# openai/Video-Pre-Training

Measured on NVIDIA H100. Metric: frames/sec MinecraftPolicy fwd, 128x128x3 BxT=128x128, higher is better.
Workload: dtype bf16

## Files before the change

video-pre-training_b200/csrc/common.cuh:

```cuda
#pragma once
#include <cuda.h>
#include <cuda_bf16.h>
#include <cuda_runtime.h>
#include <stdint.h>

#include "../../include/vpt_b200.h"

namespace vpt {

void set_error(const char* fmt, ...);
#define VPT_CHECK(cond, ...)                 \
    do {                                     \
        if (!(cond)) {                       \
            vpt::set_error(__VA_ARGS__);     \
            return VPT_ERR_ARG;              \
        }                                    \
    } while (0)
#define VPT_CUDA(expr)                                                                   \
    do {                                                                                 \
        cudaError_t _e = (expr);                                                         \
        if (_e != cudaSuccess) {                                                         \
            vpt::set_error("%s failed: %s (%s:%d)", #expr, cudaGetErrorString(_e), __FILE__, __LINE__); \
            return VPT_ERR_CUDA;                                                         \
        }                                                                                \
    } while (0)
#define VPT_LAUNCH_CHECK() VPT_CUDA(cudaGetLastError())
static int g_pdl = 0;
template <typename... KArgs, typename... Args>
static inline void launch_k(void (*kernel)(KArgs...), dim3 grid, dim3 block, size_t smem, cudaStream_t stream, Args&&... args) {
    cudaLaunchConfig_t cfg;
    memset(&cfg, 0, sizeof(cfg));
    cfg.gridDim = grid;
    cfg.blockDim = block;
    cfg.dynamicSmemBytes = smem;
    cfg.stream = stream;
    cudaLaunchAttribute attr[1];
    attr[0].id = cudaLaunchAttributeProgrammaticStreamSerialization;
    attr[0].val.programmaticStreamSerializationAllowed = 1;
    cfg.attrs = attr;
    cfg.numAttrs = g_pdl ? 1 : 0;
    (void)cudaLaunchKernelEx(&cfg, kernel, static_cast<KArgs>(args)...);
}


#ifndef VPT_NO_WATCHDOG
__device__ unsigned int g_device_error = 0;
#endif

__device__ __forceinline__ void pdl_sync() {
    asm volatile("griddepcontrol.launch_dependents;" ::: "memory");
    asm volatile("griddepcontrol.wait;" ::: "memory");
}
__device__ __forceinline__ uint32_t smem_u32(const void* p) { return (uint32_t)__cvta_generic_to_shared(p); }
__device__ __forceinline__ int lane_id() { return threadIdx.x & 31; }

__device__ __forceinline__ float warp_sum(float v) {
#pragma unroll
    for (int o = 16; o > 0; o >>= 1) v += __shfl_xor_sync(0xffffffffu, v, o);
    return v;
}
__device__ __forceinline__ float warp_max(float v) {
#pragma unroll
    for (int o = 16; o > 0; o >>= 1) v = fmaxf(v, __shfl_xor_sync(0xffffffffu, v, o));
    return v;
}

__device__ __forceinline__ uint32_t pack_bf16(float lo, float hi) {
    __nv_bfloat162 v = __floats2bfloat162_rn(lo, hi);
    return *reinterpret_cast<uint32_t*>(&v);
}
__device__ __forceinline__ float bf16_lo(uint32_t v) { return __uint_as_float(v << 16); }
__device__ __forceinline__ float bf16_hi(uint32_t v) { return __uint_as_float(v & 0xffff0000u); }
__device__ __forceinline__ float round_bf16(float v) { return __bfloat162float(__float2bfloat16_rn(v)); }

__device__ __forceinline__ void mbar_init(uint64_t* bar, uint32_t count) {
    asm volatile("mbarrier.init.shared::cta.b64 [%0], %1;" ::"r"(smem_u32(bar)), "r"(count));
}
__device__ __forceinline__ void fence_barrier_init() { asm volatile("fence.mbarrier_init.release.cluster;" ::: "memory"); }
__device__ __forceinline__ void fence_proxy_async() { asm volatile("fence.proxy.async.shared::cta;" ::: "memory"); }
__device__ __forceinline__ void mbar_expect_tx(uint64_t* bar, uint32_t bytes) {
    asm volatile("mbarrier.arrive.expect_tx.shared::cta.b64 _, [%0], %1;" ::"r"(smem_u32(bar)), "r"(bytes) : "memory");
}
__device__ __forceinline__ void mbar_arrive(uint64_t* bar) {
    asm volatile("mbarrier.arrive.shared::cta.b64 _, [%0];" ::"r"(smem_u32(bar)) : "memory");
}
__device__ __forceinline__ bool mbar_try_wait(uint64_t* bar, uint32_t parity) {
    uint32_t ok;
    asm volatile(
        "{\n\t.reg .pred p;\n\t"
        "mbarrier.try_wait.parity.shared::cta.b64 p, [%1], %2;\n\t"
        "selp.b32 %0, 1, 0, p;\n\t}"
        : "=r"(ok)
        : "r"(smem_u32(bar)), "r"(parity)
        : "memory");
    return ok != 0;
}
__device__ __forceinline__ bool mbar_try_wait_sleep(uint64_t* bar, uint32_t parity, uint32_t ns) {
    uint32_t ok;
    asm volatile(
        "{\n\t.reg .pred p;\n\t"
        "mbarrier.try_wait.parity.shared::cta.b64 p, [%1], %2, %3;\n\t"
        "selp.b32 %0, 1, 0, p;\n\t}"
        : "=r"(ok)
        : "r"(smem_u32(bar)), "r"(parity), "r"(ns)
        : "memory");
    return ok != 0;
}
__device__ __forceinline__ bool mbar_wait(uint64_t* bar, uint32_t parity, unsigned int code) {
    if (mbar_try_wait(bar, parity)) return true;
    const long long t0 = clock64();
    for (unsigned int it = 1;; ++it) {
        if (mbar_try_wait_sleep(bar, parity, 20000u)) return true;
        if ((it & 63u) == 0u) {
            if (*(volatile unsigned int*)&g_device_error != 0u) return false;
            if (clock64() - t0 > 3000000000LL) {
                atomicCAS(&g_device_error, 0u, code);
                return false;
            }
        }
    }
}

__device__ __forceinline__ void tma_prefetch_desc(const CUtensorMap* m) {
    asm volatile("prefetch.tensormap [%0];" ::"l"((uint64_t)m) : "memory");
}
__device__ __forceinline__ void tma_load_2d(void* dst, const CUtensorMap* m, uint64_t* bar, int c0, int c1) {
    asm volatile(
        "cp.async.bulk.tensor.2d.shared::cluster.global.tile.mbarrier::complete_tx::bytes [%0], [%1, {%3, %4}], [%2];" ::"r"(
            smem_u32(dst)),
        "l"((uint64_t)m), "r"(smem_u32(bar)), "r"(c0), "r"(c1)
        : "memory");
}
__device__ __forceinline__ void tma_load_4d(void* dst, const CUtensorMap* m, uint64_t* bar, int c0, int c1, int c2, int c3) {
    asm volatile(
        "cp.async.bulk.tensor.4d.shared::cluster.global.tile.mbarrier::complete_tx::bytes [%0], [%1, {%3, %4, %5, %6}], [%2];" ::"r"(
            smem_u32(dst)),
        "l"((uint64_t)m), "r"(smem_u32(bar)), "r"(c0), "r"(c1), "r"(c2), "r"(c3)
        : "memory");
}

__device__ __forceinline__ void tma_store_2d(const CUtensorMap* m, const void* src, int c0, int c1) {
    asm volatile("cp.async.bulk.tensor.2d.global.shared::cta.bulk_group [%0, {%2, %3}], [%1];" ::"l"((uint64_t)m), "r"(smem_u32(src)), "r"(c0),
                 "r"(c1)
                 : "memory");
}
__device__ __forceinline__ void bulk_commit() { asm volatile("cp.async.bulk.commit_group;" ::: "memory"); }
template <int N>
__device__ __forceinline__ void bulk_wait_read() {
    asm volatile("cp.async.bulk.wait_group.read %0;" ::"n"(N) : "memory");
}
template <int N>
__device__ __forceinline__ void bulk_wait_all() {
    asm volatile("cp.async.bulk.wait_group %0;" ::"n"(N) : "memory");
}
__device__ __forceinline__ void named_bar_sync(int id, int nthreads) { asm volatile("bar.sync %0, %1;" ::"r"(id), "r"(nthreads) : "memory"); }
__device__ __forceinline__ void named_bar_arrive(int id, int nthreads) { asm volatile("bar.arrive %0, %1;" ::"r"(id), "r"(nthreads) : "memory"); }

__device__ __forceinline__ void tma_load_2d_mc(void* dst, const CUtensorMap* m, uint64_t* bar, int c0, int c1, uint16_t cta_mask) {
    asm volatile(
        "cp.async.bulk.tensor.2d.shared::cluster.global.tile.mbarrier::complete_tx::bytes.multicast::cluster [%0], [%1, {%3, %4}], [%2], %5;" ::"r"(
            smem_u32(dst)),
        "l"((uint64_t)m), "r"(smem_u32(bar)), "r"(c0), "r"(c1), "h"(cta_mask)
        : "memory");
}

__device__ __forceinline__ void mbar_arrive_cluster(uint64_t* bar, uint32_t rank) {
    asm volatile(
        "{\n\t.reg .b32 ra;\n\t"
        "mapa.shared::cluster.u32 ra, %0, %1;\n\t"
        "mbarrier.arrive.release.cluster.shared::cluster.b64 _, [ra];\n\t}" ::"r"(smem_u32(bar)),
        "r"(rank)
        : "memory");
}
__device__ __forceinline__ uint32_t cluster_ctarank() {
    uint32_t r;
    asm volatile("mov.u32 %0, %%cluster_ctarank;" : "=r"(r));
    return r;
}
__device__ __forceinline__ void cluster_sync_all() {
    asm volatile("barrier.cluster.arrive.release.aligned;\n\tbarrier.cluster.wait.acquire.aligned;" ::: "memory");
}

__device__ __forceinline__ void wgmma_fence() { asm volatile("wgmma.fence.sync.aligned;" ::: "memory"); }
__device__ __forceinline__ void wgmma_commit() { asm volatile("wgmma.commit_group.sync.aligned;" ::: "memory"); }
template <int N>
__device__ __forceinline__ void wgmma_wait() { asm volatile("wgmma.wait_group.sync.aligned %0;" ::"n"(N) : "memory"); }
template <int N>
__device__ __forceinline__ void wgmma_reg_fence(float (&d)[N]) {
#pragma unroll
    for (int i = 0; i < N; ++i) asm volatile("" : "+f"(d[i])::"memory");
}

template <int TA, int TB>
__device__ __forceinline__ void wgmma_n64(float (&d)[32], uint64_t a_desc, uint64_t b_desc, uint32_t accumulate) {
    asm volatile(
        "{\n\t.reg .pred p;\n\t"
        "setp.ne.b32 p, %34, 0;\n\t"
        "wgmma.mma_async.sync.aligned.m64n64k16.f32.bf16.bf16 "
        "{%0, %1, %2, %3, %4, %5, %6, %7, %8, %9, %10, %11, %12, %13, %14, %15, %16, %17, %18, %19, %20, %21, %22, %23, %24, %25, %26, %27, %28, %29, %30, %31}, %32, %33, p, 1, 1, %35, %36;\n\t}"
        : "+f"(d[0]), "+f"(d[1]), "+f"(d[2]), "+f"(d[3]), "+f"(d[4]), "+f"(d[5]), "+f"(d[6]), "+f"(d[7]), "+f"(d[8]), "+f"(d[9]), "+f"(d[10]), "+f"(d[11]), "+f"(d[12]), "+f"(d[13]), "+f"(d[14]), "+f"(d[15]), "+f"(d[16]), "+f"(d[17]), "+f"(d[18]), "+f"(d[19]), "+f"(d[20]), "+f"(d[21]), "+f"(d[22]), "+f"(d[23]), "+f"(d[24]), "+f"(d[25]), "+f"(d[26]), "+f"(d[27]), "+f"(d[28]), "+f"(d[29]), "+f"(d[30]), "+f"(d[31])
        : "l"(a_desc), "l"(b_desc), "r"(accumulate), "n"(TA), "n"(TB)
        : "memory");
}

template <int TA, int TB>
__device__ __forceinline__ void wgmma_n128(float (&d)[64], uint64_t a_desc, uint64_t b_desc, uint32_t accumulate) {
    asm volatile(
        "{\n\t.reg .pred p;\n\t"
        "setp.ne.b32 p, %66, 0;\n\t"
        "wgmma.mma_async.sync.aligned.m64n128k16.f32.bf16.bf16 "
        "{%0, %1, %2, %3, %4, %5, %6, %7, %8, %9, %10, %11, %12, %13, %14, %15, %16, %17, %18, %19, %20, %21, %22, %23, %24, %25, %26, %27, %28, %29, %30, %31, %32, %33, %34, %35, %36, %37, %38, %39, %40, %41, %42, %43, %44, %45, %46, %47, %48, %49, %50, %51, %52, %53, %54, %55, %56, %57, %58, %59, %60, %61, %62, %63}, %64, %65, p, 1, 1, %67, %68;\n\t}"
        : "+f"(d[0]), "+f"(d[1]), "+f"(d[2]), "+f"(d[3]), "+f"(d[4]), "+f"(d[5]), "+f"(d[6]), "+f"(d[7]), "+f"(d[8]), "+f"(d[9]), "+f"(d[10]), "+f"(d[11]), "+f"(d[12]), "+f"(d[13]), "+f"(d[14]), "+f"(d[15]), "+f"(d[16]), "+f"(d[17]), "+f"(d[18]), "+f"(d[19]), "+f"(d[20]), "+f"(d[21]), "+f"(d[22]), "+f"(d[23]), "+f"(d[24]), "+f"(d[25]), "+f"(d[26]), "+f"(d[27]), "+f"(d[28]), "+f"(d[29]), "+f"(d[30]), "+f"(d[31]), "+f"(d[32]), "+f"(d[33]), "+f"(d[34]), "+f"(d[35]), "+f"(d[36]), "+f"(d[37]), "+f"(d[38]), "+f"(d[39]), "+f"(d[40]), "+f"(d[41]), "+f"(d[42]), "+f"(d[43]), "+f"(d[44]), "+f"(d[45]), "+f"(d[46]), "+f"(d[47]), "+f"(d[48]), "+f"(d[49]), "+f"(d[50]), "+f"(d[51]), "+f"(d[52]), "+f"(d[53]), "+f"(d[54]), "+f"(d[55]), "+f"(d[56]), "+f"(d[57]), "+f"(d[58]), "+f"(d[59]), "+f"(d[60]), "+f"(d[61]), "+f"(d[62]), "+f"(d[63])
        : "l"(a_desc), "l"(b_desc), "r"(accumulate), "n"(TA), "n"(TB)
        : "memory");
}

template <int R>
__device__ __forceinline__ void setmaxnreg_dec() { asm volatile("setmaxnreg.dec.sync.aligned.u32 %0;" ::"n"(R)); }
template <int R>
__device__ __forceinline__ void setmaxnreg_inc() { asm volatile("setmaxnreg.inc.sync.aligned.u32 %0;" ::"n"(R)); }

__device__ __forceinline__ uint64_t gmma_desc_sw128(uint32_t smem_addr, uint32_t lbo_bytes = 16u, uint32_t sbo_bytes = 1024u) {
    uint64_t d = 0;
    d |= (uint64_t)((smem_addr & 0x3FFFFu) >> 4);
    d |= (uint64_t)(lbo_bytes >> 4) << 16;
    d |= (uint64_t)(sbo_bytes >> 4) << 32;
    d |= (uint64_t)1 << 62;
    return d;
}

template <int NR>
__device__ __forceinline__ void wgmma_frag_store(const float (&d)[NR], float* stg, int pitch, int col0) {
    const int w = (threadIdx.x >> 5) & 3, l = threadIdx.x & 31;
    const int r0 = 16 * w + (l >> 2), c0 = col0 + 2 * (l & 3);
#pragma unroll
    for (int i = 0; i < NR / 4; ++i) {
        *reinterpret_cast<float2*>(stg + (size_t)r0 * pitch + c0 + 8 * i) = make_float2(d[4 * i], d[4 * i + 1]);
        *reinterpret_cast<float2*>(stg + (size_t)(r0 + 8) * pitch + c0 + 8 * i) = make_float2(d[4 * i + 2], d[4 * i + 3]);
    }
}
__device__ __forceinline__ void stg_ld_32(const float* src, uint32_t (&v)[32]) {
#pragma unroll
    for (int q = 0; q < 8; ++q) {
        const float4 x = reinterpret_cast<const float4*>(src)[q];
        v[4 * q] = __float_as_uint(x.x); v[4 * q + 1] = __float_as_uint(x.y); v[4 * q + 2] = __float_as_uint(x.z); v[4 * q + 3] = __float_as_uint(x.w);
    }
}

}
```

video-pre-training_b200/csrc/conv_zp.cuh:

```cuda
#pragma once
#include "common.cuh"
#include "gemm_tc.cuh"

namespace vpt {

static int g_cz_dbg = 0;

constexpr int kCzThreads = 384;
constexpr int kCzMaxBStages = 8;
constexpr int kCzProducerRegs = 24, kCzMmaRegs = 240;

constexpr int kCzBarOrder = 1, kCzBarStg = 3, kCzBarWg = 5;

struct ConvZpParams {
    long long Q;
    int H, W, Wp, FS;
    int N, block_n, num_n_tiles, cin, cin_blocks;
    int a_box_rows, a_boxes, a_stage_bytes, b_stages;
    int dbg;
    int bo;
    long long num_m_tiles;
    const float* mr;
    const float* S1;
    const float* S2;
    int relu;
    const __nv_bfloat16* residual;
    __nv_bfloat16* out;
    float* stat_part;
    const float* Ef;
    const float* res_scale;
    const float* res_shift;
};

template <int BN>
__device__ __forceinline__ void cz_mma_k16(float (&acc)[BN / 2], uint64_t a_desc, uint64_t b_desc, uint32_t accumulate) {
    if constexpr (BN == 128)
        wgmma_n128<0, 0>(acc, a_desc, b_desc, accumulate);
    else
        wgmma_n64<0, 0>(acc, a_desc, b_desc, accumulate);
}

template <int BN>
__global__ void __launch_bounds__(kCzThreads, 1)
conv3x3_zp_kernel(const __grid_constant__ CUtensorMap tmA, const __grid_constant__ CUtensorMap tmB, const ConvZpParams p) {
    static_assert(BN == 64 || BN == 128, "BN is 64 or 128");
    pdl_sync();
    extern __shared__ uint8_t smem_raw[];
    const uint32_t raw = smem_u32(smem_raw);
    uint8_t* smem = smem_raw + (((raw + 1023u) & ~1023u) - raw);
    constexpr uint32_t b_stage_bytes = (uint32_t)BN * kBlockK * 2;
    uint8_t* smem_a = smem;
    uint8_t* smem_b = smem + 2 * (size_t)p.a_stage_bytes;
    float* stg = reinterpret_cast<float*>(smem_b + (size_t)p.b_stages * b_stage_bytes);
    uint64_t* bars = reinterpret_cast<uint64_t*>(reinterpret_cast<uint8_t*>(stg) + kStgBytes);
    uint64_t* a_full = bars;
    uint64_t* a_empty = bars + 2;
    uint64_t* b_full = bars + 4;
    uint64_t* b_empty = bars + 4 + kCzMaxBStages;

    const int warp = threadIdx.x >> 5;
    const int lane = threadIdx.x & 31;

    if (warp == 8 && lane == 0) {
        tma_prefetch_desc(&tmA);
        tma_prefetch_desc(&tmB);
        for (int i = 0; i < 2; ++i) {
            mbar_init(&a_full[i], 1);
            mbar_init(&a_empty[i], 1);
        }
        for (int i = 0; i < p.b_stages; ++i) {
            mbar_init(&b_full[i], 1);
            mbar_init(&b_empty[i], 1);
        }
        fence_barrier_init();
    }
    __syncthreads();

    const int num_tiles = (int)(p.num_m_tiles * p.num_n_tiles);
    const int tile_begin = (int)blockIdx.x;
    const int tile_step = (int)gridDim.x;
    const int halo = p.Wp + 1;

    if (warp >= 8) {
        setmaxnreg_dec<kCzProducerRegs>();
        if (warp == 8 && lane == 0) {
            int stage = 0;
            uint32_t phase = 0;
            bool ok = true;
            for (int tile = tile_begin; tile < num_tiles && ok; tile += tile_step) {
                const int m_tile = tile / p.num_n_tiles;
                const int span0 = m_tile * kBlockM - halo;
                for (int cb = 0; cb < p.cin_blocks; ++cb) {
                    if (!(ok = mbar_wait(&a_empty[stage], phase ^ 1u, 0x110u))) break;
                    mbar_expect_tx(&a_full[stage], (uint32_t)p.a_stage_bytes);
                    uint8_t* sa = smem_a + (size_t)stage * p.a_stage_bytes;
                    for (int b = 0; b < p.a_boxes; ++b)
                        tma_load_2d(sa + (size_t)b * p.a_box_rows * 128, &tmA, &a_full[stage], cb * kBlockK, span0 + b * p.a_box_rows);
                    advance(stage, phase, 2);
                }
            }
        } else if (warp == 9 && lane == 0) {
            int stage = 0;
            uint32_t phase = 0;
            bool ok = true;
            for (int tile = tile_begin; tile < num_tiles && ok; tile += tile_step) {
                const int n0 = (tile % p.num_n_tiles) * BN;
                for (int cb = 0; cb < p.cin_blocks && ok; ++cb) {
                    for (int tap = 0; tap < 9; ++tap) {
                        if (!(ok = mbar_wait(&b_empty[stage], phase ^ 1u, 0x120u))) break;
                        mbar_expect_tx(&b_full[stage], b_stage_bytes);
                        tma_load_2d(smem_b + (size_t)stage * b_stage_bytes, &tmB, &b_full[stage], tap * p.cin + cb * kBlockK, n0);
                        advance(stage, phase, p.b_stages);
                    }
                }
            }
        }
        return;
    }

    setmaxnreg_inc<kCzMmaRegs>();
    const int wg = warp >> 2;
    const int wwarp = warp & 3;
    float* my_row = stg + (size_t)(wwarp * 32 + lane) * kStgPitch;
    const int nchunks = BN >> 5;
    const int c_half = (nchunks + 1) >> 1;
    const int P = p.num_n_tiles * 2;
    const bool res_vec = (((uintptr_t)p.residual | (uintptr_t)p.res_scale | (uintptr_t)p.res_shift) & 15) == 0;
    const int b_per_tile = 9 * p.cin_blocks;
    for (int s = wg; tile_begin + s * tile_step < num_tiles; s += 2) {
        const int tile = tile_begin + s * tile_step;
        const bool has_next = tile + tile_step < num_tiles;
        const int m_tile = tile / p.num_n_tiles;
        const int n_tile = tile % p.num_n_tiles;
        const int n0 = n_tile * BN;
        const long long a_it = (long long)s * p.cin_blocks, b_it = (long long)s * b_per_tile;
        int astage = (int)(a_it & 1), bstage = (int)(b_it % p.b_stages);
        uint32_t aphase = (uint32_t)((a_it >> 1) & 1), bphase = (uint32_t)((b_it / p.b_stages) & 1);

        if (s > 0) named_bar_sync(kCzBarOrder + wg, 256);
        float frag[2][BN / 2];
        bool ok = true;
        int prev_b = -1, prev_a = -1;
        for (int cb = 0; cb < p.cin_blocks && ok; ++cb) {
            if (!(ok = mbar_wait(&a_full[astage], aphase, 0x310u))) break;
            const uint32_t a_base = smem_u32(smem_a + (size_t)astage * p.a_stage_bytes);
#pragma unroll 1
            for (int tap = 0; tap < 9; ++tap) {
                if (!(ok = mbar_wait(&b_full[bstage], bphase, 0x320u))) break;
                const uint32_t b_addr = smem_u32(smem_b + (size_t)bstage * b_stage_bytes);
                const int row_off = (tap / 3) * p.Wp + (tap % 3);
                const uint32_t a_addr = a_base + (uint32_t)row_off * 128u;
                const uint64_t a_bo = p.bo ? ((uint64_t)((a_addr >> 7) & 7u) << 49) : 0ull;
                wgmma_fence();
#pragma unroll
                for (int k = 0; k < kBlockK / 16; ++k) {
                    const uint32_t acc = (uint32_t)((cb | tap | k) != 0);
                    const uint64_t bd = gmma_desc_sw128(b_addr + k * 32);
                    cz_mma_k16<BN>(frag[0], gmma_desc_sw128(a_addr + k * 32) | a_bo, bd, acc);
                    cz_mma_k16<BN>(frag[1], gmma_desc_sw128(a_addr + 64u * 128u + k * 32) | a_bo, bd, acc);
                }
                wgmma_commit();
                wgmma_wait<1>();
                if ((threadIdx.x & 127) == 0) {
                    if (prev_b >= 0) mbar_arrive(&b_empty[prev_b]);
                    if (prev_a >= 0) mbar_arrive(&a_empty[prev_a]);
                }
                prev_a = -1;
                prev_b = bstage;
                advance(bstage, bphase, p.b_stages);
            }
            prev_a = astage;
            advance(astage, aphase, 2);
        }
        if (has_next) named_bar_arrive(kCzBarOrder + (wg ^ 1), 256);
        wgmma_wait<0>();
#pragma unroll
        for (int h = 0; h < 2; ++h) wgmma_reg_fence(frag[h]);
        if ((threadIdx.x & 127) == 0) {
            if (prev_b >= 0) mbar_arrive(&b_empty[prev_b]);
            if (prev_a >= 0) mbar_arrive(&a_empty[prev_a]);
        }
        if (!ok) {
            if (has_next) named_bar_arrive(kCzBarStg + (wg ^ 1), 256);
            break;
        }

        if (s > 0) named_bar_sync(kCzBarStg + wg, 256);
#pragma unroll
        for (int h = 0; h < 2; ++h) wgmma_frag_store(frag[h], stg + (size_t)h * 64 * kStgPitch, kStgPitch, 0);
        named_bar_sync(kCzBarWg + wg, 128);

        const int q = m_tile * kBlockM + wwarp * 32 + lane;
        const bool row_ok = q < p.Q;
        const int f = q / p.FS;
        const int r = q - f * p.FS;
        const int y = r / p.Wp, x = r - y * p.Wp;
        const bool interior = row_ok && (y < p.H) && (x < p.W);
        float ga = 1.f, gb = 0.f;
        if (p.mr != nullptr && interior) {
            const float mean = __ldg(p.mr + 2 * f), rstd = __ldg(p.mr + 2 * f + 1);
            ga = rstd;
            gb = rstd * mean;
        }
        const int cy = (y == 0) ? 0 : ((y == p.H - 1) ? 2 : 1);
        const int cx = (x == 0) ? 0 : ((x == p.W - 1) ? 2 : 1);
        const int cls = interior ? cy * 3 + cx : 0;
        const float* s1row = p.S1 ? p.S1 + (size_t)cls * p.N : nullptr;
        const float* s2row = p.S2 ? p.S2 + (size_t)cls * p.N : nullptr;
        if (p.Ef) {
            s1row = nullptr;
            s2row = p.Ef + ((size_t)(interior ? f : 0) * 9 + cls) * p.N;
        }
        const float* rarow = (p.res_scale && interior) ? p.res_scale + (size_t)f * p.N : nullptr;
        const float* rbrow = (p.res_scale && interior) ? p.res_shift + (size_t)f * p.N : nullptr;
        float st_s0 = 0.f, st_ss0 = 0.f, st_s1 = 0.f, st_ss1 = 0.f;

        const int qw = m_tile * kBlockM + wwarp * 32;
        float* wrows = stg + (size_t)(wwarp * 32) * kStgPitch;
        const int seg = lane & 3;
#pragma unroll 1
        for (int c = 0; c < (p.dbg == 2 ? 0 : nchunks); ++c) {
            const int g = c < c_half ? 0 : 1;
            const int nb = n0 + c * 32;
            const int lim = min(32, min(BN - c * 32, p.N - nb));
            if (lim <= 0) break;
            const bool full = (lim == 32) && ((p.N & 7) == 0) && res_vec;
            uint32_t acc[32];
            float v[32];
            uint32_t pk[16];
            if (full) {
                stg_ld_32(my_row + c * 32, acc);
                __syncwarp();
                if (p.residual != nullptr) {
#pragma unroll
                    for (int k = 0; k < 4; ++k) {
                        const int rr = 8 * k + (lane >> 2);
                        if (qw + rr < p.Q)
                            reinterpret_cast<uint4*>(wrows + (size_t)rr * kStgPitch + c * 32)[seg] =
                                __ldg(reinterpret_cast<const uint4*>(p.residual + (size_t)(qw + rr) * p.N + nb) + seg);
                    }
                    __syncwarp();
                }
                if (row_ok) {
                    if (!interior) {
#pragma unroll
                        for (int j = 0; j < 16; ++j) pk[j] = 0u;
                    } else {
#pragma unroll
                        for (int qq = 0; qq < 8; ++qq) {
                            float4 a1 = s1row ? __ldg(reinterpret_cast<const float4*>(s1row + nb) + qq) : make_float4(0, 0, 0, 0);
                            float4 a2 = s2row ? __ldg(reinterpret_cast<const float4*>(s2row + nb) + qq) : make_float4(0, 0, 0, 0);
                            v[4 * qq + 0] = fmaf(ga, __uint_as_float(acc[4 * qq + 0]), fmaf(-gb, a1.x, a2.x));
                            v[4 * qq + 1] = fmaf(ga, __uint_as_float(acc[4 * qq + 1]), fmaf(-gb, a1.y, a2.y));
                            v[4 * qq + 2] = fmaf(ga, __uint_as_float(acc[4 * qq + 2]), fmaf(-gb, a1.z, a2.z));
                            v[4 * qq + 3] = fmaf(ga, __uint_as_float(acc[4 * qq + 3]), fmaf(-gb, a1.w, a2.w));
                        }
                        if (p.relu == 1) {
#pragma unroll
                            for (int j = 0; j < 32; ++j) v[j] = fmaxf(v[j], 0.f);
                        }
                        if (p.residual != nullptr) {
                            const uint4* rp = reinterpret_cast<const uint4*>(my_row + c * 32);
#pragma unroll
                            for (int qq = 0; qq < 4; ++qq) {
                                const uint4 rr = rp[qq];
                                const float r8[8] = {bf16_lo(rr.x), bf16_hi(rr.x), bf16_lo(rr.y), bf16_hi(rr.y),
                                                     bf16_lo(rr.z), bf16_hi(rr.z), bf16_lo(rr.w), bf16_hi(rr.w)};
                                if (rarow) {
                                    const float4* ra4 = reinterpret_cast<const float4*>(rarow + nb) + 2 * qq;
                                    const float4* rb4 = reinterpret_cast<const float4*>(rbrow + nb) + 2 * qq;
                                    const float4 a0 = __ldg(ra4), a1 = __ldg(ra4 + 1), b0 = __ldg(rb4), b1 = __ldg(rb4 + 1);
                                    const float ra[8] = {a0.x, a0.y, a0.z, a0.w, a1.x, a1.y, a1.z, a1.w};
                                    const float rb[8] = {b0.x, b0.y, b0.z, b0.w, b1.x, b1.y, b1.z, b1.w};
#pragma unroll
                                    for (int j = 0; j < 8; ++j) v[8 * qq + j] += fmaf(ra[j], r8[j], rb[j]);
                                } else {
#pragma unroll
                                    for (int j = 0; j < 8; ++j) v[8 * qq + j] += r8[j];
                                }
                            }
                        }
                        if (p.relu == 2) {
#pragma unroll
                            for (int j = 0; j < 32; ++j) v[j] = fmaxf(v[j], 0.f);
                        }
#pragma unroll
                        for (int j = 0; j < 16; ++j) pk[j] = pack_bf16(v[2 * j], v[2 * j + 1]);
                        if (p.stat_part) {
                            float s_ = g ? st_s1 : st_s0, ss_ = g ? st_ss1 : st_ss0;
#pragma unroll
                            for (int j = 0; j < 16; ++j) {
                                const float lo = bf16_lo(pk[j]), hi = bf16_hi(pk[j]);
                                s_ += lo; ss_ = fmaf(lo, lo, ss_);
                                s_ += hi; ss_ = fmaf(hi, hi, ss_);
                            }
                            if (g) { st_s1 = s_; st_ss1 = ss_; } else { st_s0 = s_; st_ss0 = ss_; }
                        }
                    }
#pragma unroll
                    for (int qq = 0; qq < 4; ++qq)
                        reinterpret_cast<uint4*>(my_row + c * 32 + 16)[qq] = make_uint4(pk[4 * qq], pk[4 * qq + 1], pk[4 * qq + 2], pk[4 * qq + 3]);
                }
                __syncwarp();
                if (p.dbg != 1) {
#pragma unroll
                    for (int k = 0; k < 4; ++k) {
                        const int rr = 8 * k + (lane >> 2);
                        if (qw + rr < p.Q)
                            reinterpret_cast<uint4*>(p.out + (size_t)(qw + rr) * p.N + nb)[seg] =
                                reinterpret_cast<const uint4*>(wrows + (size_t)rr * kStgPitch + c * 32 + 16)[seg];
                    }
                }
                continue;
            }
            if (!row_ok) continue;
            stg_ld_32(my_row + c * 32, acc);
            __nv_bfloat16* op = p.out + (size_t)q * p.N + nb;
            if (!interior) {
                for (int j = 0; j < lim; ++j) op[j] = __float2bfloat16_rn(0.f);
                continue;
            }
#pragma unroll
            for (int j = 0; j < 32; ++j) {
                float a1 = 0.f, a2 = 0.f;
                if (j < lim) {
                    if (s1row) a1 = __ldg(s1row + nb + j);
                    if (s2row) a2 = __ldg(s2row + nb + j);
                }
                v[j] = fmaf(ga, __uint_as_float(acc[j]), fmaf(-gb, a1, a2));
            }
            if (p.relu == 1) {
#pragma unroll
                for (int j = 0; j < 32; ++j) v[j] = fmaxf(v[j], 0.f);
            }
            if (p.residual != nullptr) {
                const __nv_bfloat16* rp = p.residual + (size_t)q * p.N + nb;
#pragma unroll
                for (int j = 0; j < 32; ++j)
                    if (j < lim) v[j] += rarow ? fmaf(__ldg(rarow + nb + j), __bfloat162float(rp[j]), __ldg(rbrow + nb + j)) : __bfloat162float(rp[j]);
            }
            if (p.relu == 2) {
#pragma unroll
                for (int j = 0; j < 32; ++j) v[j] = fmaxf(v[j], 0.f);
            }
#pragma unroll
            for (int j = 0; j < 16; ++j) pk[j] = pack_bf16(v[2 * j], v[2 * j + 1]);
            if (p.stat_part) {
                float s_ = g ? st_s1 : st_s0, ss_ = g ? st_ss1 : st_ss0;
#pragma unroll
                for (int j = 0; j < 16; ++j) {
                    const float lo = bf16_lo(pk[j]), hi = bf16_hi(pk[j]);
                    if (2 * j < lim) { s_ += lo; ss_ = fmaf(lo, lo, ss_); }
                    if (2 * j + 1 < lim) { s_ += hi; ss_ = fmaf(hi, hi, ss_); }
                }
                if (g) { st_s1 = s_; st_ss1 = ss_; } else { st_s0 = s_; st_ss0 = ss_; }
            }
            if (p.dbg != 1) {
#pragma unroll
                for (int j = 0; j < 32; ++j)
                    if (j < lim) op[j] = __float2bfloat16_rn(v[j]);
            }
        }
        if (has_next) named_bar_arrive(kCzBarStg + (wg ^ 1), 256);
        if (p.stat_part && row_ok)
            reinterpret_cast<float4*>(p.stat_part)[((size_t)q * P + n_tile * 2) >> 1] = make_float4(st_s0, st_ss0, st_s1, st_ss1);
    }
}

}

namespace vpt {
static inline void conv_zp_block_n(long long Q, int N, int* bn, int* nt) {
    choose_block_n(N, bn, nt);
    const long long tiles = (Q + kBlockM - 1) / kBlockM;
    if (tiles * *nt >= 64 || *bn == 64) return;
    *bn = 64;
    *nt = (N + 63) / 64;
}
}

extern "C" int vpt_conv3x3_zp(const vpt_conv_zp_args* a, void* stream) {
    using namespace vpt;
    VPT_CHECK(a && a->x && a->w && a->out, "vpt_conv3x3_zp: null operand");
    const int H = a->H, W = a->W, C = a->Cin, N = a->Cout;
    VPT_CHECK(a->F > 0 && H >= 2 && W >= 2 && C > 0 && C % 64 == 0 && N > 0 && N % 16 == 0,
              "vpt_conv3x3_zp: need F>0, H,W>=2, Cin %% 64 == 0, Cout %% 16 == 0 (F=%d H=%d W=%d Cin=%d Cout=%d)", a->F, H, W, C, N);
    VPT_CHECK(W <= 182, "vpt_conv3x3_zp: W=%d too wide (at most 182: two input spans of 128 + 2*(W+2) rows must fit in shared memory)", W);
    VPT_CHECK(((uintptr_t)a->x & 15) == 0 && ((uintptr_t)a->w & 15) == 0 && ((uintptr_t)a->out & 15) == 0, "vpt_conv3x3_zp: pointers must be 16-byte aligned");
    ConvZpParams p;
    memset(&p, 0, sizeof(p));
    p.H = H; p.W = W; p.Wp = W + 1; p.FS = (H + 1) * (W + 1);
    p.Q = (long long)a->F * p.FS;
    VPT_CHECK(p.Q <= 2147483647LL - kBlockM, "vpt_conv3x3_zp: too many rows for 32-bit row indices and TMA coordinates");
    p.N = N; p.cin = C; p.cin_blocks = C / 64;
    conv_zp_block_n(p.Q, N, &p.block_n, &p.num_n_tiles);
    p.num_m_tiles = (p.Q + kBlockM - 1) / kBlockM;
    const int span = kBlockM + 2 * (p.Wp + 1);
    p.a_boxes = (span + 255) / 256;
    p.a_box_rows = ((span + p.a_boxes - 1) / p.a_boxes + 7) / 8 * 8;
    VPT_CHECK(p.a_box_rows <= 256, "vpt_conv3x3_zp: span does not fit the TMA box limit");
    p.a_stage_bytes = p.a_boxes * p.a_box_rows * 128;
    const uint32_t b_stage_bytes = (uint32_t)p.block_n * kBlockK * 2;
    const size_t fixed_bytes = 1024 + 2 * (size_t)p.a_stage_bytes + kStgBytes + (4 + 2 * kCzMaxBStages) * 8;
    int bst = (int)((227 * 1024 - (long long)fixed_bytes) / b_stage_bytes);
    if (bst > kCzMaxBStages) bst = kCzMaxBStages;
    VPT_CHECK(bst >= 2, "vpt_conv3x3_zp: not enough shared memory for the weight pipeline (W=%d Cout=%d)", W, N);
    p.b_stages = bst;
    const size_t smem_bytes = fixed_bytes + (size_t)bst * b_stage_bytes;

    CUtensorMap tmA, tmB;
    {
        cuuint64_t dims[2] = {(cuuint64_t)C, (cuuint64_t)p.Q};
        cuuint64_t strides[1] = {(cuuint64_t)C * 2};
        cuuint32_t box[2] = {64, (cuuint32_t)p.a_box_rows};
        int r = make_tmap_bf16(&tmA, a->x, 2, dims, strides, box);
        if (r) return r;
    }
    {
        cuuint64_t dims[2] = {(cuuint64_t)9 * C, (cuuint64_t)N};
        cuuint64_t strides[1] = {(cuuint64_t)9 * C * 2};
        cuuint32_t box[2] = {64, (cuuint32_t)p.block_n};
        int r = make_tmap_bf16(&tmB, a->w, 2, dims, strides, box);
        if (r) return r;
    }
    VPT_CHECK(!(a->mr && !a->S1 && !a->Ef), "vpt_conv3x3_zp: mr given without S1 (or Ef)");
    VPT_CHECK(!a->Ef || a->mr, "vpt_conv3x3_zp: Ef needs mr = (0, rstd) per frame");
    VPT_CHECK(!a->res_scale == !a->res_shift && (!a->res_scale || a->residual) && (!a->res_scale || N % 8 == 0),
              "vpt_conv3x3_zp: res_scale / res_shift come as a pair, with a residual, Cout %% 8 == 0");
    p.mr = a->mr; p.S1 = a->mr ? a->S1 : nullptr; p.S2 = a->S2; p.relu = a->relu;
    p.residual = reinterpret_cast<const __nv_bfloat16*>(a->residual);
    p.out = reinterpret_cast<__nv_bfloat16*>(a->out);
    p.stat_part = a->stat_part;
    p.Ef = a->Ef; p.res_scale = a->res_scale; p.res_shift = a->res_shift;
    p.dbg = g_cz_dbg;
    p.bo = g_dbg_bo > 0 ? 1 : 0;

    static bool attr_set = false;
    if (!attr_set) {
        VPT_CUDA(cudaFuncSetAttribute(conv3x3_zp_kernel<64>, cudaFuncAttributeMaxDynamicSharedMemorySize, 227 * 1024));
        VPT_CUDA(cudaFuncSetAttribute(conv3x3_zp_kernel<128>, cudaFuncAttributeMaxDynamicSharedMemorySize, 227 * 1024));
        attr_set = true;
    }
    const long long tiles = p.num_m_tiles * p.num_n_tiles;
    long long grid = num_sms();
    if (grid <= 0) grid = 132;
    if (grid > tiles) grid = tiles;
    if (p.block_n == 64)
        launch_k(conv3x3_zp_kernel<64>, dim3((unsigned)grid), dim3(kCzThreads), smem_bytes, (cudaStream_t)stream, tmA, tmB, p);
    else
        launch_k(conv3x3_zp_kernel<128>, dim3((unsigned)grid), dim3(kCzThreads), smem_bytes, (cudaStream_t)stream, tmA, tmB, p);
    VPT_LAUNCH_CHECK();
    return VPT_OK;
}

extern "C" int vpt_set_conv_pair_mode(int32_t on) {
    vpt::g_cz_dbg = (on & 0xff) >> 4;
    return VPT_OK;
}

extern "C" int vpt_set_conv_swap_mode(int32_t on) {
    (void)on;
    return VPT_OK;
}

extern "C" int64_t vpt_conv_zp_t_stat_floats(int32_t F, int32_t H, int32_t W, int32_t Cout) {
    (void)F; (void)H; (void)W; (void)Cout;
    return 0;
}

extern "C" int vpt_conv_zp_t_stats_finalize(const float* part, float* mr, int32_t F, int32_t H, int32_t W, float eps, void* stream) {
    (void)part; (void)mr; (void)F; (void)H; (void)W; (void)eps; (void)stream;
    vpt::set_error("vpt_conv_zp_t_stats_finalize: no convolution kernel of this build emits per-tile partials (vpt_conv_zp_t_stat_floats is 0)");
    return VPT_ERR_ARG;
}

extern "C" int vpt_conv_zp_stat_parts(int32_t F, int32_t H, int32_t W, int32_t Cout) {
    const long long Q = (long long)F * (H + 1) * (W + 1);
    int bn, nt;
    vpt::conv_zp_block_n(Q, Cout, &bn, &nt);
    return nt * 2;
}
```

Baseline: 26620.

## Stage conv epilogue per warp and chunk instead of whole-tile shared staging

The epilogue of the zero-padded 3x3 conv kernel now gives each warp a private 32-row staging area with a 36-float pitch. Each 32-column chunk of the wgmma fragment is written there on demand, instead of staging the whole tile into a buffer shared by the warpgroup. This removes the inter-warpgroup staging barriers and the warpgroup-wide sync, and shrinks the staging shared memory, which can leave room for more weight pipeline stages. Residual loads for the next chunk are issued early, before the wgmma wait and between chunks, to hide global latency. The cost is more __syncwarp calls, a switch on chunk index, and more live registers for the prefetched residual.

```diff
diff --git a/video-pre-training_b200/csrc/common.cuh b/video-pre-training_b200/csrc/common.cuh
--- a/video-pre-training_b200/csrc/common.cuh
+++ b/video-pre-training_b200/csrc/common.cuh
@@ -239,6 +239,17 @@
         *reinterpret_cast<float2*>(stg + (size_t)(r0 + 8) * pitch + c0 + 8 * i) = make_float2(d[4 * i + 2], d[4 * i + 3]);
     }
 }
+template <int C, int NR>
+__device__ __forceinline__ void wgmma_frag_store_chunk(const float (&d)[NR], float* blk, int pitch) {
+    static_assert(16 * C + 16 <= NR, "chunk outside the fragment");
+    const int l = threadIdx.x & 31;
+    float* dst = blk + (size_t)(l >> 2) * pitch + 2 * (l & 3);
+#pragma unroll
+    for (int i = 0; i < 4; ++i) {
+        *reinterpret_cast<float2*>(dst + 8 * i) = make_float2(d[16 * C + 4 * i], d[16 * C + 4 * i + 1]);
+        *reinterpret_cast<float2*>(dst + (size_t)8 * pitch + 8 * i) = make_float2(d[16 * C + 4 * i + 2], d[16 * C + 4 * i + 3]);
+    }
+}
 __device__ __forceinline__ void stg_ld_32(const float* src, uint32_t (&v)[32]) {
 #pragma unroll
     for (int q = 0; q < 8; ++q) {
diff --git a/video-pre-training_b200/csrc/conv_zp.cuh b/video-pre-training_b200/csrc/conv_zp.cuh
--- a/video-pre-training_b200/csrc/conv_zp.cuh
+++ b/video-pre-training_b200/csrc/conv_zp.cuh
@@ -10,7 +10,10 @@
 constexpr int kCzMaxBStages = 8;
 constexpr int kCzProducerRegs = 24, kCzMmaRegs = 240;
 
-constexpr int kCzBarOrder = 1, kCzBarStg = 3, kCzBarWg = 5;
+constexpr int kCzBarOrder = 1;
+
+constexpr int kCzStgPitch = 36;
+constexpr uint32_t kCzStgBytes = 8u * 32u * kCzStgPitch * 4u;
 
 struct ConvZpParams {
     long long Q;
@@ -41,6 +44,20 @@
 }
 
 template <int BN>
+__device__ __forceinline__ void cz_stage_chunk(const float (&frag)[2][BN / 2], int c, float* wrows) {
+#pragma unroll
+    for (int h = 0; h < 2; ++h) {
+        float* blk = wrows + (size_t)h * 16 * kCzStgPitch;
+        switch (c) {
+            case 0: wgmma_frag_store_chunk<0>(frag[h], blk, kCzStgPitch); break;
+            case 1: wgmma_frag_store_chunk<1>(frag[h], blk, kCzStgPitch); break;
+            case 2: if constexpr (BN == 128) wgmma_frag_store_chunk<2>(frag[h], blk, kCzStgPitch); break;
+            case 3: if constexpr (BN == 128) wgmma_frag_store_chunk<3>(frag[h], blk, kCzStgPitch); break;
+        }
+    }
+}
+
+template <int BN>
 __global__ void __launch_bounds__(kCzThreads, 1)
 conv3x3_zp_kernel(const __grid_constant__ CUtensorMap tmA, const __grid_constant__ CUtensorMap tmB, const ConvZpParams p) {
     static_assert(BN == 64 || BN == 128, "BN is 64 or 128");
@@ -52,16 +69,15 @@
     uint8_t* smem_a = smem;
     uint8_t* smem_b = smem + 2 * (size_t)p.a_stage_bytes;
     float* stg = reinterpret_cast<float*>(smem_b + (size_t)p.b_stages * b_stage_bytes);
-    uint64_t* bars = reinterpret_cast<uint64_t*>(reinterpret_cast<uint8_t*>(stg) + kStgBytes);
+    uint64_t* bars = reinterpret_cast<uint64_t*>(reinterpret_cast<uint8_t*>(stg) + kCzStgBytes);
     uint64_t* a_full = bars;
     uint64_t* a_empty = bars + 2;
     uint64_t* b_full = bars + 4;
     uint64_t* b_empty = bars + 4 + kCzMaxBStages;
 
     const int warp = threadIdx.x >> 5;
-    const int lane = threadIdx.x & 31;
-
-    if (warp == 8 && lane == 0) {
+
+    if (threadIdx.x == 8 * 32) {
         tma_prefetch_desc(&tmA);
         tma_prefetch_desc(&tmB);
         for (int i = 0; i < 2; ++i) {
@@ -83,7 +99,7 @@
 
     if (warp >= 8) {
         setmaxnreg_dec<kCzProducerRegs>();
-        if (warp == 8 && lane == 0) {
+        if (threadIdx.x == 8 * 32) {
             int stage = 0;
             uint32_t phase = 0;
             bool ok = true;
@@ -99,7 +115,7 @@
                     advance(stage, phase, 2);
                 }
             }
-        } else if (warp == 9 && lane == 0) {
+        } else if (threadIdx.x == 9 * 32) {
             int stage = 0;
             uint32_t phase = 0;
             bool ok = true;
@@ -120,12 +136,19 @@
 
     setmaxnreg_inc<kCzMmaRegs>();
     const int wg = warp >> 2;
-    const int wwarp = warp & 3;
-    float* my_row = stg + (size_t)(wwarp * 32 + lane) * kStgPitch;
-    const int nchunks = BN >> 5;
-    const int c_half = (nchunks + 1) >> 1;
+    const int lane = threadIdx.x & 31;
+    const int wrow0 = (warp & 3) * 16;
+    float* wrows = stg + (size_t)warp * 32 * kCzStgPitch;
+    float* my_row = wrows + (size_t)lane * kCzStgPitch;
+    const int my_trow = ((lane >> 4) << 6) + wrow0 + (lane & 15);
+    const int seg = lane & 3;
+    const int seg_row0 = lane >> 2, seg_trow0 = wrow0 + seg_row0;
+    const auto seg_row = [&](int k) { return seg_row0 + 8 * k; };
+    const auto seg_trow = [&](int k) { return seg_trow0 + ((k >> 1) << 6) + ((k & 1) << 3); };
+    constexpr int nchunks = BN >> 5;
+    constexpr int c_half = (nchunks + 1) >> 1;
     const int P = p.num_n_tiles * 2;
-    const bool res_vec = (((uintptr_t)p.residual | (uintptr_t)p.res_scale | (uintptr_t)p.res_shift) & 15) == 0;
+    const bool res_vec = ((p.N & 7) == 0) && (((uintptr_t)p.residual | (uintptr_t)p.res_scale | (uintptr_t)p.res_shift) & 15) == 0;
     const int b_per_tile = 9 * p.cin_blocks;
     for (int s = wg; tile_begin + s * tile_step < num_tiles; s += 2) {
         const int tile = tile_begin + s * tile_step;
@@ -173,6 +196,19 @@
             advance(astage, aphase, 2);
         }
         if (has_next) named_bar_arrive(kCzBarOrder + (wg ^ 1), 256);
+
+        const int q0 = m_tile * kBlockM;
+        const auto chunk_full = [&](int c) { return p.N - (n0 + c * 32) >= 32 && res_vec; };
+        uint4 res_next[4];
+        const auto res_load = [&](int c) {
+#pragma unroll
+            for (int k = 0; k < 4; ++k)
+                res_next[k] = q0 + seg_trow(k) < p.Q
+                                  ? __ldg(reinterpret_cast<const uint4*>(p.residual + (size_t)(q0 + seg_trow(k)) * p.N + n0 + c * 32) + seg)
+                                  : make_uint4(0u, 0u, 0u, 0u);
+        };
+        if (p.residual != nullptr && p.dbg != 2 && chunk_full(0)) res_load(0);
+
         wgmma_wait<0>();
 #pragma unroll
         for (int h = 0; h < 2; ++h) wgmma_reg_fence(frag[h]);
@@ -180,17 +216,9 @@
             if (prev_b >= 0) mbar_arrive(&b_empty[prev_b]);
             if (prev_a >= 0) mbar_arrive(&a_empty[prev_a]);
         }
-        if (!ok) {
-            if (has_next) named_bar_arrive(kCzBarStg + (wg ^ 1), 256);
-            break;
-        }
-
-        if (s > 0) named_bar_sync(kCzBarStg + wg, 256);
-#pragma unroll
-        for (int h = 0; h < 2; ++h) wgmma_frag_store(frag[h], stg + (size_t)h * 64 * kStgPitch, kStgPitch, 0);
-        named_bar_sync(kCzBarWg + wg, 128);
-
-        const int q = m_tile * kBlockM + wwarp * 32 + lane;
+        if (!ok) break;
+
+        const int q = q0 + my_trow;
         const bool row_ok = q < p.Q;
         const int f = q / p.FS;
         const int r = q - f * p.FS;
@@ -215,106 +243,101 @@
         const float* rbrow = (p.res_scale && interior) ? p.res_shift + (size_t)f * p.N : nullptr;
         float st_s0 = 0.f, st_ss0 = 0.f, st_s1 = 0.f, st_ss1 = 0.f;
 
-        const int qw = m_tile * kBlockM + wwarp * 32;
-        float* wrows = stg + (size_t)(wwarp * 32) * kStgPitch;
-        const int seg = lane & 3;
 #pragma unroll 1
         for (int c = 0; c < (p.dbg == 2 ? 0 : nchunks); ++c) {
             const int g = c < c_half ? 0 : 1;
             const int nb = n0 + c * 32;
-            const int lim = min(32, min(BN - c * 32, p.N - nb));
+            const int lim = min(32, p.N - nb);
             if (lim <= 0) break;
-            const bool full = (lim == 32) && ((p.N & 7) == 0) && res_vec;
+            const bool full = chunk_full(c);
             uint32_t acc[32];
-            float v[32];
-            uint32_t pk[16];
+            __syncwarp();
+            cz_stage_chunk<BN>(frag, c, wrows);
+            __syncwarp();
+            stg_ld_32(my_row, acc);
             if (full) {
-                stg_ld_32(my_row + c * 32, acc);
                 __syncwarp();
                 if (p.residual != nullptr) {
 #pragma unroll
-                    for (int k = 0; k < 4; ++k) {
-                        const int rr = 8 * k + (lane >> 2);
-                        if (qw + rr < p.Q)
-                            reinterpret_cast<uint4*>(wrows + (size_t)rr * kStgPitch + c * 32)[seg] =
-                                __ldg(reinterpret_cast<const uint4*>(p.residual + (size_t)(qw + rr) * p.N + nb) + seg);
-                    }
+                    for (int k = 0; k < 4; ++k)
+                        if (q0 + seg_trow(k) < p.Q) reinterpret_cast<uint4*>(wrows + (size_t)seg_row(k) * kCzStgPitch)[seg] = res_next[k];
+                    if (c + 1 < nchunks && chunk_full(c + 1)) res_load(c + 1);
                     __syncwarp();
                 }
                 if (row_ok) {
+                    uint4* dst = reinterpret_cast<uint4*>(my_row + 16);
                     if (!interior) {
 #pragma unroll
-                        for (int j = 0; j < 16; ++j) pk[j] = 0u;
+                        for (int o = 0; o < 4; ++o) dst[o] = make_uint4(0u, 0u, 0u, 0u);
                     } else {
-#pragma unroll
-                        for (int qq = 0; qq < 8; ++qq) {
-                            float4 a1 = s1row ? __ldg(reinterpret_cast<const float4*>(s1row + nb) + qq) : make_float4(0, 0, 0, 0);
-                            float4 a2 = s2row ? __ldg(reinterpret_cast<const float4*>(s2row + nb) + qq) : make_float4(0, 0, 0, 0);
-                            v[4 * qq + 0] = fmaf(ga, __uint_as_float(acc[4 * qq + 0]), fmaf(-gb, a1.x, a2.x));
-                            v[4 * qq + 1] = fmaf(ga, __uint_as_float(acc[4 * qq + 1]), fmaf(-gb, a1.y, a2.y));
-                            v[4 * qq + 2] = fmaf(ga, __uint_as_float(acc[4 * qq + 2]), fmaf(-gb, a1.z, a2.z));
-                            v[4 * qq + 3] = fmaf(ga, __uint_as_float(acc[4 * qq + 3]), fmaf(-gb, a1.w, a2.w));
-                        }
-                        if (p.relu == 1) {
-#pragma unroll
-                            for (int j = 0; j < 32; ++j) v[j] = fmaxf(v[j], 0.f);
-                        }
-                        if (p.residual != nullptr) {
-                            const uint4* rp = reinterpret_cast<const uint4*>(my_row + c * 32);
-#pragma unroll
-                            for (int qq = 0; qq < 4; ++qq) {
-                                const uint4 rr = rp[qq];
+                        float s_ = g ? st_s1 : st_s0, ss_ = g ? st_ss1 : st_ss0;
+#pragma unroll
+                        for (int o = 0; o < 4; ++o) {
+                            float v[8];
+#pragma unroll
+                            for (int h = 0; h < 2; ++h) {
+                                const int qq = 2 * o + h;
+                                float4 a1 = s1row ? __ldg(reinterpret_cast<const float4*>(s1row + nb) + qq) : make_float4(0, 0, 0, 0);
+                                float4 a2 = s2row ? __ldg(reinterpret_cast<const float4*>(s2row + nb) + qq) : make_float4(0, 0, 0, 0);
+                                v[4 * h + 0] = fmaf(ga, __uint_as_float(acc[4 * qq + 0]), fmaf(-gb, a1.x, a2.x));
+                                v[4 * h + 1] = fmaf(ga, __uint_as_float(acc[4 * qq + 1]), fmaf(-gb, a1.y, a2.y));
+                                v[4 * h + 2] = fmaf(ga, __uint_as_float(acc[4 * qq + 2]), fmaf(-gb, a1.z, a2.z));
+                                v[4 * h + 3] = fmaf(ga, __uint_as_float(acc[4 * qq + 3]), fmaf(-gb, a1.w, a2.w));
+                            }
+                            if (p.relu == 1) {
+#pragma unroll
+                                for (int j = 0; j < 8; ++j) v[j] = fmaxf(v[j], 0.f);
+                            }
+                            if (p.residual != nullptr) {
+                                const uint4 rr = reinterpret_cast<const uint4*>(my_row)[o];
                                 const float r8[8] = {bf16_lo(rr.x), bf16_hi(rr.x), bf16_lo(rr.y), bf16_hi(rr.y),
                                                      bf16_lo(rr.z), bf16_hi(rr.z), bf16_lo(rr.w), bf16_hi(rr.w)};
                                 if (rarow) {
-                                    const float4* ra4 = reinterpret_cast<const float4*>(rarow + nb) + 2 * qq;
-                                    const float4* rb4 = reinterpret_cast<const float4*>(rbrow + nb) + 2 * qq;
+                                    const float4* ra4 = reinterpret_cast<const float4*>(rarow + nb) + 2 * o;
+                                    const float4* rb4 = reinterpret_cast<const float4*>(rbrow + nb) + 2 * o;
                                     const float4 a0 = __ldg(ra4), a1 = __ldg(ra4 + 1), b0 = __ldg(rb4), b1 = __ldg(rb4 + 1);
                                     const float ra[8] = {a0.x, a0.y, a0.z, a0.w, a1.x, a1.y, a1.z, a1.w};
                                     const float rb[8] = {b0.x, b0.y, b0.z, b0.w, b1.x, b1.y, b1.z, b1.w};
 #pragma unroll
-                                    for (int j = 0; j < 8; ++j) v[8 * qq + j] += fmaf(ra[j], r8[j], rb[j]);
+                                    for (int j = 0; j < 8; ++j) v[j] += fmaf(ra[j], r8[j], rb[j]);
                                 } else {
 #pragma unroll
-                                    for (int j = 0; j < 8; ++j) v[8 * qq + j] += r8[j];
+                                    for (int j = 0; j < 8; ++j) v[j] += r8[j];
                                 }
                             }
+                            if (p.relu == 2) {
+#pragma unroll
+                                for (int j = 0; j < 8; ++j) v[j] = fmaxf(v[j], 0.f);
+                            }
+                            uint32_t pk[4];
+#pragma unroll
+                            for (int j = 0; j < 4; ++j) pk[j] = pack_bf16(v[2 * j], v[2 * j + 1]);
+                            if (p.stat_part) {
+#pragma unroll
+                                for (int j = 0; j < 4; ++j) {
+                                    const float lo = bf16_lo(pk[j]), hi = bf16_hi(pk[j]);
+                                    s_ += lo; ss_ = fmaf(lo, lo, ss_);
+                                    s_ += hi; ss_ = fmaf(hi, hi, ss_);
+                                }
+                            }
+                            dst[o] = make_uint4(pk[0], pk[1], pk[2], pk[3]);
                         }
-                        if (p.relu == 2) {
-#pragma unroll
-                            for (int j = 0; j < 32; ++j) v[j] = fmaxf(v[j], 0.f);
-                        }
-#pragma unroll
-                        for (int j = 0; j < 16; ++j) pk[j] = pack_bf16(v[2 * j], v[2 * j + 1]);
-                        if (p.stat_part) {
-                            float s_ = g ? st_s1 : st_s0, ss_ = g ? st_ss1 : st_ss0;
-#pragma unroll
-                            for (int j = 0; j < 16; ++j) {
-                                const float lo = bf16_lo(pk[j]), hi = bf16_hi(pk[j]);
-                                s_ += lo; ss_ = fmaf(lo, lo, ss_);
-                                s_ += hi; ss_ = fmaf(hi, hi, ss_);
-                            }
-                            if (g) { st_s1 = s_; st_ss1 = ss_; } else { st_s0 = s_; st_ss0 = ss_; }
-                        }
+                        if (g) { st_s1 = s_; st_ss1 = ss_; } else { st_s0 = s_; st_ss0 = ss_; }
                     }
-#pragma unroll
-                    for (int qq = 0; qq < 4; ++qq)
-                        reinterpret_cast<uint4*>(my_row + c * 32 + 16)[qq] = make_uint4(pk[4 * qq], pk[4 * qq + 1], pk[4 * qq + 2], pk[4 * qq + 3]);
                 }
                 __syncwarp();
                 if (p.dbg != 1) {
 #pragma unroll
-                    for (int k = 0; k < 4; ++k) {
-                        const int rr = 8 * k + (lane >> 2);
-                        if (qw + rr < p.Q)
-                            reinterpret_cast<uint4*>(p.out + (size_t)(qw + rr) * p.N + nb)[seg] =
-                                reinterpret_cast<const uint4*>(wrows + (size_t)rr * kStgPitch + c * 32 + 16)[seg];
-                    }
+                    for (int k = 0; k < 4; ++k)
+                        if (q0 + seg_trow(k) < p.Q)
+                            reinterpret_cast<uint4*>(p.out + (size_t)(q0 + seg_trow(k)) * p.N + nb)[seg] =
+                                reinterpret_cast<const uint4*>(wrows + (size_t)seg_row(k) * kCzStgPitch + 16)[seg];
                 }
                 continue;
             }
             if (!row_ok) continue;
-            stg_ld_32(my_row + c * 32, acc);
+            float v[32];
+            uint32_t pk[16];
             __nv_bfloat16* op = p.out + (size_t)q * p.N + nb;
             if (!interior) {
                 for (int j = 0; j < lim; ++j) op[j] = __float2bfloat16_rn(0.f);
@@ -361,7 +384,6 @@
                     if (j < lim) op[j] = __float2bfloat16_rn(v[j]);
             }
         }
-        if (has_next) named_bar_arrive(kCzBarStg + (wg ^ 1), 256);
         if (p.stat_part && row_ok)
             reinterpret_cast<float4*>(p.stat_part)[((size_t)q * P + n_tile * 2) >> 1] = make_float4(st_s0, st_ss0, st_s1, st_ss1);
     }
@@ -401,7 +423,7 @@
     VPT_CHECK(p.a_box_rows <= 256, "vpt_conv3x3_zp: span does not fit the TMA box limit");
     p.a_stage_bytes = p.a_boxes * p.a_box_rows * 128;
     const uint32_t b_stage_bytes = (uint32_t)p.block_n * kBlockK * 2;
-    const size_t fixed_bytes = 1024 + 2 * (size_t)p.a_stage_bytes + kStgBytes + (4 + 2 * kCzMaxBStages) * 8;
+    const size_t fixed_bytes = 1024 + 2 * (size_t)p.a_stage_bytes + kCzStgBytes + (4 + 2 * kCzMaxBStages) * 8;
     int bst = (int)((227 * 1024 - (long long)fixed_bytes) / b_stage_bytes);
     if (bst > kCzMaxBStages) bst = kCzMaxBStages;
     VPT_CHECK(bst >= 2, "vpt_conv3x3_zp: not enough shared memory for the weight pipeline (W=%d Cout=%d)", W, N);
```

After: 27960, median of 6. 5.0% higher.
